# ilias-laoukili/gnn-sparsification-research

Hardware: AMD Instinct MI355X
Metric: scored edges/sec (Jaccard+ApproxER) (higher is better)
Workload: dtype f64; 1 GPU; configs[1] Roman-empire Jaccard+ApproxER; n=22662, E=65854, jl_k=2674, cg_maxiter=500, blas_threads_order=8, rng=device, parallelism=1 GPU

## Files before the change

### gnn-sparsification-research_amd/csrc/gs_cg.hpp

```cpp
#pragma once
#include <algorithm>
#include <climits>
#include <cstddef>
#include <cstdlib>

#include "gs_internal.hpp"

namespace gs {

static constexpr int kMaxChunks = 64;
static constexpr int64_t kStoreQRowLen = 8;

struct ChunkArg {
    int32_t count;
    int64_t a[kMaxChunks];
    int64_t len[kMaxChunks];
};
static_assert(offsetof(ChunkArg, len) == offsetof(ChunkArg, a) + sizeof(int64_t) * kMaxChunks,
              "chunks_to_device copies a and len as one block");

inline ChunkArg make_chunks(int64_t n, int32_t threads) {
    ChunkArg ch{};
    if (n <= 10000 || threads <= 1) {
        ch.count = 1;
// ... 160 lines not shown
    int64_t slots;
    bool slots_forced;
    bool res_unit;
    bool res_dcount;
    bool res_prof;
    bool res_ell;
    bool res_stab;
    bool res_qlds;
    int res_rbw;
    int reg_nt;
    int64_t reg_keep;
    int reg_split;
    bool reg_split_auto;
    int32_t reg_split_spin;
    int reg_window;
};

bool cg_regres_applies(int64_t n, int T, const int64_t *len, int reg_nt);
bool cg_regres_wide(int64_t n, int T, const int64_t *len, int reg_nt);

static constexpr int kRegLayoutChunks = 16;
static constexpr size_t kRegLdsBytes = 160 * 1024;

inline int reg_geometry(int NT, int T, const int64_t *len, int &G) {
    if (T < 1 || 32 * T > NT) return -1;
    G = 1;
    while (G < 8 && 32 * T * (2 * G) <= NT) G *= 2;
    int64_t smax = 0;
    for (int t = 0; t < T; ++t) smax = std::max<int64_t>(smax, (len[t] & ~(int64_t)31) >> 5);
    return (int)((smax + G - 1) / G);
// ... 68 lines not shown
    int64_t zs = 0;
    for (int t = 0; t < T; ++t) {
        L.lbase[t] = zs;
        zs += L.keep[t];
    }
    L.W = W;
    for (int t = 0; t < T && W > 0; ++t) {
        L.wbase[t] = zs;
        zs += W * align;
    }
    L.zslot = zs;
    L.dyn = sizeof(double) * ((size_t)zs + 2 + L.dsl + 6 * (size_t)nch + 2 * kRegLayoutChunks);
    return true;
}

inline CgPlan cg_plan(int64_t n, int64_t lnnz, int64_t ncols, int32_t blas_threads) {
    CgPlan p{};
    if (blas_threads > kMaxChunks) blas_threads = kMaxChunks;
    p.ch = make_chunks(n, blas_threads);
    const ChunkArg &ch = p.ch;

    const char *e;
    p.res_unit = !(e = getenv("GSPARSE_RES_UNIT")) || atoi(e) != 0;
    p.res_dcount = !(e = getenv("GSPARSE_RES_DCOUNT")) || atoi(e) != 0;
    p.res_prof = getenv("GSPARSE_RES_PROF") != nullptr;
    p.res_ell = (e = getenv("GSPARSE_RES_ELL")) && atoi(e) != 0;
    p.res_stab = !(e = getenv("GSPARSE_RES_STAB")) || atoi(e) != 0;
    p.res_qlds = !(e = getenv("GSPARSE_RES_QLDS")) || atoi(e) != 0;
    p.res_rbw = 0;
    if ((e = getenv("GSPARSE_RES_RBW")))
        p.res_rbw = atoi(e) == 44 ? 44 : atoi(e) == 27 ? 27 : atoi(e) == 26 ? 26 : 28;
    p.reg_nt = ((e = getenv("GSPARSE_REG_NT")) && atoi(e) == 256) ? 256 : 512;
    p.reg_keep = (e = getenv("GSPARSE_REG_KEEP")) ? atoll(e) : INT64_MAX;
    p.reg_split = (e = getenv("GSPARSE_REG_SPLIT")) ? atoi(e) : -1;
    p.reg_split_auto = getenv("GSPARSE_REG_SPLIT_AUTO") != nullptr;
    p.reg_split_spin = (e = getenv("GSPARSE_REG_SPLIT_SPIN")) ? atoi(e) : INT32_MIN;
    p.reg_window = -1;
    if ((e = getenv("GSPARSE_REG_WINDOW"))) p.reg_window = atoi(e) == 3 ? 3 : atoi(e) == 4 ? 4 : 0;

    const int64_t waves2 = ((ncols + 127) / 128) * 32 * (int64_t)ch.count;
    p.cpl = waves2 >= 4096 ? 2 : 1;
    if ((e = getenv("GSPARSE_CG_CPL"))) p.cpl = atoi(e) == 1 ? 1 : 2;
    const int64_t ncb = (int32_t)((ncols + 64 * p.cpl - 1) / (64 * p.cpl));

    const bool resident = n > 10000 && n <= 24576 && ch.count >= 4 && lnnz <= kStoreQRowLen * n;
    const bool regres = cg_regres_applies(n, ch.count, ch.len, p.reg_nt);
    const bool regwide = cg_regres_wide(n, ch.count, ch.len, p.reg_nt);
    p.mode = resident && regwide                   ? 5
             : resident                            ? 4
             : (n > 0 && lnnz > kStoreQRowLen * n) ? 3
             : ncols >= 2048                       ? 0
             : ncols >= 512                        ? 1
                                                   : 3;
// ... 49 lines not shown
```

### gnn-sparsification-research_amd/csrc/gs_cg_reg.hip

```cpp
#include "gs_cg.hpp"
#include "gs_cg_reg.hpp"

#ifndef GS_CG_XG
#define GS_CG_XG 0
#endif

namespace gs {

__global__ void k_ell8_count(int32_t n, const int64_t *__restrict__ lp, int64_t *__restrict__ cnt,
                             uint16_t *__restrict__ rlen) {
    for (int64_t i = blockIdx.x * (int64_t)blockDim.x + threadIdx.x; i < n;
         i += (int64_t)gridDim.x * blockDim.x) {
        const int64_t len = lp[i + 1] - lp[i];
        cnt[i] = len > 8 ? len - 8 : 0;
        rlen[i] = (uint16_t)len;
    }
}

__device__ __forceinline__ uint32_t p_code(int32_t c, int32_t i, int T, const int64_t *__restrict__ tab,
                                           int W, int &nwin) {
    if (c < tab[0] || c >= tab[T - 1] + tab[kRegMaxChunks + T - 1]) return 0x8000u | (uint32_t)c;
    int t = 0;
    while (t + 1 < T && c >= tab[t + 1]) ++t;
    const int64_t o = c - tab[t], keep = tab[2 * kRegMaxChunks + t];
    if (o < keep) return (uint32_t)(tab[3 * kRegMaxChunks + t] + o);
    if (W > 0) {
        const int64_t oi = (int64_t)i - tab[t], n32 = tab[kRegMaxChunks + t] & ~(int64_t)31;
        if (oi >= 0 && oi < n32 && o < n32) {
            const int64_t sc = o >> 6, si = oi >> 6;
            if (sc - si <= 1 && si - sc <= 1) {
                ++nwin;
                return (uint32_t)(tab[4 * kRegMaxChunks + t] + ((sc - (keep >> 6)) % W) * 64 + (o & 63));
            }
        }
    }
    return 0x8000u | (uint32_t)c;
}

__device__ __forceinline__ int row_dslot(int32_t c, int T, const int64_t *__restrict__ tab, int G,
                                         int dmul, int32_t d0 = 0) {
    int t = 0;
    while (t + 1 < T && c >= tab[t + 1]) ++t;
// ... 5 lines not shown
    const int tid = (chain / CW) * 64 + (chain % CW) + CW * g;
    if (dmul == 3) {
        const int lb = (int)tab[3 * kRegMaxChunks + t];
        const int s0 = d0 + (tid & ~31);
        return (tid & ~31) + ((lb + (tid & 31) + 1 - s0) & 31);
    }
    return dmul == 2 ? 2 * tid + par : tid;
}

__global__ void k_ell8_fill(int32_t r0, int32_t n, int T, const int64_t *__restrict__ tab, uint32_t pad,
                            int G, int dmul, int32_t dslot0, const int64_t *__restrict__ lp,
                            const int32_t *__restrict__ li, const double *__restrict__ lv,
                            const int64_t *__restrict__ optr, uint4 *__restrict__ ell,
                            double *__restrict__ ellv, uint16_t *__restrict__ ocol,
                            double *__restrict__ oval, uint8_t *__restrict__ rflag, int W,
                            unsigned long long *__restrict__ wcount) {
    for (int64_t i = r0 + blockIdx.x * (int64_t)blockDim.x + threadIdx.x; i < n;
         i += (int64_t)gridDim.x * blockDim.x) {
        const int64_t e0 = lp[i], len = lp[i + 1] - e0;
        const uint32_t dcode = dslot0 >= 0 ? (uint32_t)(dslot0 + row_dslot((int32_t)i, T, tab, G, dmul, dslot0)) : 0u;
        int nwin = 0;
        auto code = [&](int64_t e) -> uint32_t {
            return (dslot0 >= 0 && li[e] == i) ? dcode : p_code(li[e], (int32_t)i, T, tab, W, nwin);
        };
        uint32_t w[4] = {0, 0, 0, 0};
        bool glob = false;
        for (int k = 0; k < 8; ++k) {
            const uint32_t cc = k < len ? code(e0 + k) : pad;
            glob = glob || (cc & 0x8000u) != 0;
            w[k >> 1] |= cc << (16 * (k & 1));
            if (ellv) ellv[i * 8 + k] = k < len ? lv[e0 + k] : 0.0;
        }
        ell[i] = make_uint4(w[0], w[1], w[2], w[3]);
        if (rflag) rflag[i] = (uint8_t)((glob ? 1 : 0) | (len > 8 ? 2 : 0));
        for (int64_t k = 8; k < len; ++k) {
            ocol[optr[i] + k - 8] = (uint16_t)code(e0 + k);
            if (oval) oval[optr[i] + k - 8] = lv[e0 + k];
        }
// ... 32 lines not shown
    hipStream_t s = c->stream;
    const int T = plan.ch.count;
    const int64_t *ha = plan.ch.a, *hlen = plan.ch.len;
    const int64_t slots = plan.slots;
    const bool ufast = unit && dcount;
    RegLayout lay0, layw;
    GS_CHECK(reg_layout(n, plan.ch, plan.reg_nt, plan.reg_keep, ufast, lay0), GS_EUNSUPPORTED,
             "register-resident CG: n=%lld, %d chunks out of range", (long long)n, T);
    const int NT = lay0.NT, G = lay0.G, rsel = lay0.R;
    const int wask = !kRegWindowBuilt ? 0 : plan.reg_window < 0 ? kRegWindowDefault : plan.reg_window;
    const bool have_w = wask > 0 && reg_layout(n, plan.ch, plan.reg_nt, plan.reg_keep, ufast, layw, wask) &&
                        layw.W > 0;
    const bool dbank = GS_CG_V2 && NT == 512 && G == 2 && ufast;
    const int dsl = lay0.dsl;
    const size_t lds_max = kRegLdsBytes;
    double regv = c->er.reg;
    int64_t regbits;
    memcpy(&regbits, &regv, sizeof(regbits));
    std::vector<int64_t> key = {c->g.epoch, regbits, n, T, G, NT, ufast ? 1 : 0, unit, dcount, dbank ? 1 : 0,
                                have_w ? layw.W : 0, plan.reg_window};
    for (int t = 0; t < T; ++t) key.insert(key.end(), {ha[t], hlen[t], lay0.keep[t]});
    auto *ocnt = (int64_t *)c->buf("er_reg_ocnt").ensure(sizeof(int64_t) * (n + 1));
    auto *optr = (int64_t *)c->buf("er_reg_optr").ensure(sizeof(int64_t) * (n + 1));
    auto *rlen = (uint16_t *)c->buf("er_reg_rlen").ensure(sizeof(uint16_t) * n);
    const bool fresh = key != c->reg_ell_key;
    if (fresh) {
        c->reg_ell_key.clear();
        c->reg_split_key.clear();
        GS_HIP(hipMemsetAsync(ocnt, 0, sizeof(int64_t) * (n + 1), s));
        k_ell8_count<<<grid_for(n, 256, 8192), 256, 0, s>>>((int32_t)n, lp, ocnt, rlen);
        exclusive_scan_i64(c, ocnt, optr, n + 1);
        GS_HIP(hipMemcpyAsync(&c->reg_nov, optr + n, sizeof(int64_t), hipMemcpyDeviceToHost, s));
        GS_HIP(hipStreamSynchronize(s));
    }
    const int64_t nov = c->reg_nov;
// ... 3 lines not shown
        host.assign(5 * kRegMaxChunks, 0);
        for (int t = 0; t < T; ++t) {
            host[t] = ha[t];
            host[kRegMaxChunks + t] = hlen[t];
            host[2 * kRegMaxChunks + t] = L.keep[t];
            host[3 * kRegMaxChunks + t] = L.lbase[t];
            host[4 * kRegMaxChunks + t] = L.wbase[t];
        }
        GS_HIP(hipMemcpyAsync(dev, host.data(), kTabBytes, hipMemcpyHostToDevice, s));
    };
    auto *ell = (uint4 *)c->buf("er_reg_ell").ensure(sizeof(uint4) * n);
    auto *rflag = (uint8_t *)c->buf("er_reg_rflag").ensure((size_t)n + 64);
    double *ellv = ufast ? nullptr : (double *)c->buf("er_reg_ellv").ensure(sizeof(double) * 8 * n);
    auto *ocol = (uint16_t *)c->buf("er_reg_ocol").ensure(sizeof(uint16_t) * (nov + 1));
    double *oval = ufast ? nullptr : (double *)c->buf("er_reg_oval").ensure(sizeof(double) * (nov + 1));
    auto fill = [&](const RegLayout &L, const int64_t *dev, unsigned long long *wcount) {
        k_ell8_fill<<<grid_for(n, 256, 8192), 256, 0, s>>>(0, (int32_t)n, T, dev, (uint32_t)L.zslot, G,
                                                          NT == 256 ? 2 : dbank ? 3 : 1,
                                                          ufast ? (int32_t)L.zslot + 2 : -1,
                                                          lp, li, lv, optr, ell, ellv, ocol, oval, rflag, L.W,
                                                          wcount);
        GS_HIP(hipGetLastError());
    };
    if (fresh && have_w) {
        auto *dch2 = (int64_t *)c->buf("er_reg_chunks2").ensure(kTabBytes);
        auto *dcnt = (unsigned long long *)c->buf("er_reg_wcnt").ensure(sizeof(unsigned long long) * 3);
        unsigned long long hcnt[3] = {0, 0, 0};
        GS_HIP(hipMemsetAsync(dcnt, 0, sizeof(hcnt), s));
        upload(lay0, c->reg_hch2, dch2);
        fill(lay0, dch2, nullptr);
        k_reg_slow_slots<<<T, 64, 0, s>>>(T, dch2, rflag, dcnt);
        upload(layw, c->reg_hch, dch);
        fill(layw, dch, dcnt + 2);
        k_reg_slow_slots<<<T, 64, 0, s>>>(T, dch, rflag, dcnt + 1);
        GS_HIP(hipGetLastError());
        GS_HIP(hipMemcpyAsync(hcnt, dcnt, sizeof(hcnt), hipMemcpyDeviceToHost, s));
        GS_HIP(hipStreamSynchronize(s));
        const bool use_w = plan.reg_window > 0 || hcnt[1] < hcnt[0];
        c->reg_win[0] = use_w ? layw.W : 0;
        c->reg_win[1] = (int64_t)hcnt[0];
        c->reg_win[2] = (int64_t)hcnt[1];
        c->reg_win[3] = use_w ? (int64_t)hcnt[2] : 0;
        if (!use_w) {
            upload(lay0, c->reg_hch, dch);
            fill(lay0, dch, nullptr);
        }
        c->reg_ell_key = key;
    } else if (fresh) {
        c->reg_win[0] = 0, c->reg_win[1] = c->reg_win[2] = -1, c->reg_win[3] = 0;
        upload(lay0, c->reg_hch, dch);
        fill(lay0, dch, nullptr);
        c->reg_ell_key = key;
    }
    const RegLayout &lay = (have_w && c->reg_win[0] > 0) ? layw : lay0;
    if (!fresh) upload(lay, c->reg_hch, dch);
    const uint32_t pad = (uint32_t)lay.zslot;
    const size_t dyn = lay.dyn;
    RegArgs A{};
    A.qreg = 0;
    int ncu = 256;
    GS_HIP(hipDeviceGetAttribute(&ncu, hipDeviceAttributeMultiprocessorCount, c->device));
    int P = 0;
    int64_t W = ncols;
    split_abort_poll(c, false);
    if (c->reg_split_off && c->reg_split_off_epoch != c->g.epoch) c->reg_split_off = false;
    if (NT == 512 && T >= 2 && ncols > 0 && !c->reg_split_off) {
// ... 58 lines not shown
    A.oval = oval;
    A.diag = diag;
    A.rflag = rflag;

    A.zslot = (int32_t)pad;
    A.maxiter = maxiter;
    A.rtol = rtol;
    A.iters = iters;
    A.T = T;
    A.ca = dch;
    A.cl = dch + kRegMaxChunks;
    A.ck = dch + 2 * kRegMaxChunks;
    A.cb = dch + 3 * kRegMaxChunks;
    A.cw = dch + 4 * kRegMaxChunks;
    A.W = lay.W;
    A.prof = prof;
    auto launch_whole = [&]() {
        if (W <= 0) return;
        if (NT == 512) {
            if (G == 1) regwide_launch_g1(A, rsel, ufast, dyn, (unsigned)wslots, s);
            else if (G == 2) regwide_launch_g2(A, rsel, ufast, dyn, (unsigned)wslots, s);
            else if (G == 4) regwide_launch_g4(A, rsel, ufast, dyn, (unsigned)wslots, s);
            else regwide_launch_g8(A, rsel, ufast, dyn, (unsigned)wslots, s);
        } else if (G == 1) regres_launch_g1(A, rsel, ufast, dyn, (unsigned)wslots, s);
        else if (G == 2) regres_launch_g2(A, rsel, ufast, dyn, (unsigned)wslots, s);
        else if (G == 4) regres_launch_g4(A, rsel, ufast, dyn, (unsigned)wslots, s);
        else regres_launch_g8(A, rsel, ufast, dyn, (unsigned)wslots, s);
        GS_HIP(hipGetLastError());
    };
    if (P < 2) {
// ... 31 lines not shown
    GS_HIP(hipMemcpyAsync(dpt, c->reg_split_hpt.data(), sizeof(hpt), hipMemcpyHostToDevice, s));
    GS_HIP(hipMemcpyAsync(dtab, c->reg_split_htab.data(), sizeof(htab), hipMemcpyHostToDevice, s));
    auto *ells = (uint4 *)c->buf("er_reg_split_ell").ensure(sizeof(uint4) * n);
    double *ellvs = ufast ? nullptr : (double *)c->buf("er_reg_split_ellv").ensure(sizeof(double) * 8 * n);
    auto *ocols = (uint16_t *)c->buf("er_reg_split_ocol").ensure(sizeof(uint16_t) * (nov + 1));
    double *ovals = ufast ? nullptr : (double *)c->buf("er_reg_split_oval").ensure(sizeof(double) * (nov + 1));
    std::vector<int64_t> skey = {P, Gs};
    skey.insert(skey.end(), pc0, pc0 + P + 1);
    const bool sfresh = skey != c->reg_split_key;
    for (int h = 0; h < P && sfresh; ++h) {
        const int32_t r0 = (int32_t)ha[pc0[h]];
        const int32_t r1 = (int32_t)(ha[pc0[h + 1] - 1] + hlen[pc0[h + 1] - 1]);
        const int32_t zsh = hpt[h * kRegPartTab + 4 * kRegMaxChunks + 1];
        k_ell8_fill<<<grid_for(r1 - r0, 256, 8192), 256, 0, s>>>(
            r0, r1, pc0[h + 1] - pc0[h], dtab + h * 4 * kRegMaxChunks, (uint32_t)zsh, Gs, 1,
            ufast ? zsh + 2 : -1, lp, li, lv, optr, ells, ellvs, ocols, ovals, nullptr, 0, nullptr);
        GS_HIP(hipGetLastError());
    }
    c->reg_split_key = skey;
    double *pgs = (double *)c->buf("er_reg_split_pg").ensure(sizeof(double) * (size_t)groups * 2 * ldn);
    double *xch = (double *)c->buf("er_reg_split_xch").ensure(sizeof(double) * (size_t)groups * 2 * kRegMaxChunks);
    auto *flg = (int32_t *)c->buf("er_reg_split_flags").ensure(sizeof(int32_t) * ((size_t)groups * P + 1));
    GS_HIP(hipMemsetAsync(flg, 0, sizeof(int32_t) * ((size_t)groups * P + 1), s));
    RegArgs B = A;
    B.col0 = col0 + W;
    B.ncols = tailn;
    B.Xc = Xc + W * ldn;
    B.pg = pgs;
    B.ell = ells;
    B.ellv = ellvs;
    B.ocol = ocols;
    B.oval = ovals;
    B.prof = nullptr;
    B.P = P;
    B.ptab = dpt;
    B.xch = xch;
    B.flags = flg;
    B.abortf = flg + (size_t)groups * P;
    int wclk_khz = 100000;
    GS_HIP(hipDeviceGetAttribute(&wclk_khz, hipDeviceAttributeWallClockRate, c->device));
    B.spinmax = 20 * std::max(wclk_khz, 1);
    if (plan.reg_split_spin != INT32_MIN) B.spinmax = plan.reg_split_spin;
    const unsigned grid = (unsigned)(groups * P);
    launch_whole();
    if (Gs == 4) regwide_split_launch_g4(B, Rs, ufast, dyns, grid, s);
    else regwide_split_launch_g8(B, Rs, ufast, dyns, grid, s);
    GS_HIP(hipGetLastError());
    RegArgs Cw = A;
    Cw.col0 = col0 + W;
// ... 54 lines not shown
```

### gnn-sparsification-research_amd/csrc/gs_cg_reg.hpp

```cpp
#pragma once
#include <algorithm>

#include "gs_internal.hpp"

namespace gs {

static constexpr int kRegThreads = 512;
static constexpr int kRegMaxChunks = kRegThreads / 32;
#ifndef GS_KPRE
#define GS_KPRE 1
#endif
static constexpr int kPre = GS_KPRE;
#ifndef GS_KPRE_P
#define GS_KPRE_P GS_KPRE
#endif
static constexpr int kPreP = GS_KPRE_P;
#ifndef GS_CG_V2
#define GS_CG_V2 1
#endif
#ifndef GS_PGRP
#define GS_PGRP 4
#endif
#ifndef GS_P1S
#define GS_P1S 1
// ... 27 lines not shown
    const int64_t *ca, *cl;
    const int64_t *ck, *cb;
    long long *prof;
    int32_t qreg;
    int32_t P;
    const int32_t *ptab;
    double *xch;
    int32_t *flags;
    int32_t *abortf;
    int32_t spinmax;
    const double *diag;
    const uint8_t *rflag;
    const int32_t *gate;
    int32_t W;
    const int64_t *cw;
};
#ifndef GS_CG_QS
#define GS_CG_QS 1
#endif
#ifndef GS_CG_XG
#define GS_CG_XG 0
#endif
static constexpr bool kRegWindowBuilt = GS_CG_V2 && GS_CG_QS && !GS_CG_XG;
static constexpr int kRegWindowDefault = 3;
static constexpr int kRegPartTab = 4 * kRegMaxChunks + 4;

struct AgD {
    uint32_t lo, hi;
};
__device__ __forceinline__ double ag_get(const AgD &a) {
// ... 470 lines not shown
```

### gnn-sparsification-research_amd/csrc/gs_cg_wide.hpp

```cpp
#pragma once
#include "gs_cg_reg.hpp"

#ifndef GS_CG_QS
#define GS_CG_QS 1
#endif
#ifndef GS_CG_QPRE
#define GS_CG_QPRE 8
#endif
#ifndef GS_CG_QAUX
#define GS_CG_QAUX 2
#endif
#ifndef GS_CG_XAUX
#define GS_CG_XAUX 0
#endif
#ifndef GS_CG_XG
#define GS_CG_XG 0
#endif

namespace gs {

template <int HI>
__device__ __forceinline__ uint32_t wide_code_addr(uint32_t w) {
    uint32_t a;
    if (HI)
// ... 16 lines not shown
__device__ __forceinline__ double wide_readlane(double v, int ln) {
    const uint64_t b = (uint64_t)__double_as_longlong(v);
    const uint32_t lo = (uint32_t)__builtin_amdgcn_readlane((int)(uint32_t)b, ln);
    const uint32_t hi = (uint32_t)__builtin_amdgcn_readlane((int)(uint32_t)(b >> 32), ln);
    return __longlong_as_double((long long)(((uint64_t)hi << 32) | lo));
}

template <int G, int R, bool UNIT, bool QR, bool SPLIT = false, bool WIN = false>
__global__ void __launch_bounds__(kRegThreads) k_cg_regwide(RegArgs A) {
    constexpr int CW = 64 / G;
    constexpr bool V2 = GS_CG_V2 && UNIT && !SPLIT;
    constexpr bool DBANK = V2 && G == 2;
    constexpr bool QS = GS_CG_QS && !QR && !SPLIT;
    constexpr bool QSX = GS_CG_XG && QR && !SPLIT;
    constexpr bool P1 = GS_P1S && WIN;
    static_assert(!WIN || (V2 && G == 2 && QS),
                  "the p window: whole columns, unit form, two threads per chain, q stored");
    extern __shared__ double lds[];
    const int part = SPLIT ? (int)(blockIdx.x % (unsigned)A.P) : 0;
    const int group = SPLIT ? (int)(blockIdx.x / (unsigned)A.P) : (int)blockIdx.x;
    const int ngroups = SPLIT ? (int)(gridDim.x / (unsigned)A.P) : (int)gridDim.x;
    const int32_t *ptab = SPLIT ? A.ptab + part * kRegPartTab : nullptr;
    const int T = SPLIT ? ptab[4 * kRegMaxChunks] : A.T, nch = 32 * T;
    const int zslot = SPLIT ? ptab[4 * kRegMaxChunks + 1] : A.zslot;
    const int t0g = SPLIT ? ptab[4 * kRegMaxChunks + 2] : 0;
    const int Tg = SPLIT ? A.T : T;
    double *sp = lds;
    double *acc_pq = lds + zslot + 2 + (UNIT ? kRegThreads : 0), *acc_rr = acc_pq + nch;
    double *side_p = acc_pq + 2 * nch, *side_q = acc_pq + 3 * nch, *side_r = acc_pq + 4 * nch;
    double *side_x = acc_pq + 5 * nch;
// ... 14 lines not shown
    const int chain = (tid >> 6) * CW + jj;
    const bool live = chain < nch;
    const int t = live ? chain >> 5 : 0, j = chain & 31;
    const int L = s_ch[kRegMaxChunks + t];
    const int n32 = L & ~31;
    const int S = live ? n32 >> 5 : -1;
    const int tl = L - n32;
    int base = s_ch[t] + j + 32 * g;
    int uc = S > g ? (S - g + G - 1) / G : 0;
    const bool tail = live && g == 0 && j < tl;
    const int trow = s_ch[t] + n32 + j;
    const int tix = t * 32 + j;
    int ulds = 0;
    uint64_t gmask = 0, lmask = 0;
    uint32_t wdelta = 0, wbytes = 0;
    auto launder = [&]() {
        asm volatile("" : "+v"(base), "+v"(uc), "+s"(ulds));
        if constexpr (V2) asm volatile("" : "+s"(gmask), "+s"(lmask));
        if constexpr (WIN) asm volatile("" : "+s"(wdelta), "+s"(wbytes));
    };
    auto chunk_num = [&](int v) { return WIN ? __builtin_amdgcn_readfirstlane(v) : v; };
    const int ca_t = chunk_num(s_ch[t]), keep_t = chunk_num(s_ch[2 * kRegMaxChunks + t]),
              lbase_t = chunk_num(s_ch[3 * kRegMaxChunks + t]);
    {
        int uk = R;
        if (live) {
            const int o0 = base - ca_t;
            uk = keep_t > o0 ? (keep_t - o0 + 32 * G - 1) / (32 * G) : 0;
        }
        for (int off = 32; off >= 1; off >>= 1) uk = min(uk, __shfl_xor(uk, off, 64));
        ulds = __builtin_amdgcn_readfirstlane(uk);
    }
    auto lds0 = [&]() -> uint32_t { return (uint32_t)(lbase_t + base - ca_t) * 8u; };
    if constexpr (WIN) {
// ... 10 lines not shown
    constexpr int kOob = (int)0x80000000;
    constexpr int kAux = SPLIT ? 16 : 0;
    int poff = 0;
    auto vm_drain = [] { __builtin_amdgcn_s_waitcnt(0x0f70); };
    const __amdgpu_buffer_rsrc_t ers =
        __builtin_amdgcn_make_buffer_rsrc((void *)A.ell, 0, (int)(A.n * 16), 0x00020000);
    const __amdgpu_buffer_rsrc_t lrs =
        __builtin_amdgcn_make_buffer_rsrc((void *)A.rlen, 0, (int)(A.n * 2), 0x00020000);
    const __amdgpu_buffer_rsrc_t drs =
        __builtin_amdgcn_make_buffer_rsrc((void *)(V2 ? A.diag : nullptr), 0, (int)(V2 ? A.n * 8 : 0),
                                          0x00020000);
    if (tid == 0) spl[zslot] = 0.0;

    auto code_of = [&](int row) {
        const int o = row - ca_t;
        return o < keep_t ? lbase_t + o : 0x8000 | row;
    };
    auto ldc = [&](int cd) -> double {
        double v = spl[cd < 0x8000 ? cd : zslot];
        if (__builtin_amdgcn_ballot_w64(cd >= 0x8000)) {
            const double vg = __builtin_bit_cast(
                double, __builtin_amdgcn_raw_buffer_load_b64(prs, cd < 0x8000 ? kOob : (cd & 0x7fff) * 8 + poff, 0, kAux));
            v = cd < 0x8000 ? v : vg;
            vm_drain();
        }
        return v;
    };
    auto stc = [&](int cd, double v) {
        spl[cd < 0x8000 ? cd : zslot + 1] = v;
        if (__builtin_amdgcn_ballot_w64(cd >= 0x8000))
            __builtin_amdgcn_raw_buffer_store_b64(
// ... 361 lines not shown
                __builtin_bit_cast(__attribute__((ext_vector_type(2))) unsigned, v), xrs,
                valid(u) ? base * 8 : kOob, 256 * G * u, GS_CG_QAUX);
        };
        {
            launder();
            double acc = 0.0;
#pragma unroll
            for (int u = 0; u < R; ++u) {
                if constexpr (!QR) x[u] = 0.0;
                else qr[u] = 0.0;
                r[u] = valid(u) ? A.Rr[(int64_t)rowof(u) * A.ld + c] : 0.0;
                chain_step(acc, r[u], r[u], u, true);
            }
            if (g == 0 && live) acc_rr[chain] = acc;
            if (tail) {
                side_r[tix] = A.Rr[(int64_t)trow * A.ld + c];
                side_x[tix] = 0.0;
            }
        }
        __syncthreads();
        double rr = finish(acc_rr, side_r, side_r);
        const double bn = __builtin_sqrt(rr);
        const double atol = A.rtol * bn;
        int32_t done = 0;
        double rho_prev = 0.0, alpha_prev = 0.0;
        const bool act = !(bn == 0.0) && !(__builtin_sqrt(rr) < atol);
        for (int32_t it = 0; act && it < A.maxiter; ++it) {
            if (it > 0 && __builtin_sqrt(rr) < atol) break;
            const double rho_cur = rr;
            const double beta = it > 0 ? rho_cur / rho_prev : 0.0;
            if constexpr (SPLIT) poff = (it & 1) * (int)A.ldn * 8;
// ... 230 lines not shown
                            wq = wq == wbytes ? 0u : wq;
                        }
                    } else if constexpr (V2) {
                        if (valid(u)) qv = spmv2(rowof(u), eb[u], db[u], pv, u, pnx, png);
                    } else if (valid(u)) qv = spmv(rowof(u), eb[u], lb[u], pv, u);
                    if constexpr (QSX) q2store(u, qv);
                    else if constexpr (QR) qr[u] = qv;
                    if constexpr (QS) qstore(u, qv);
                    chain_step(acc, pv, qv, u);
                    __builtin_amdgcn_sched_barrier(0);
                }
                if (g == 0 && live) acc_pq[chain] = acc;
                if (tail) {
                    double pt;
                    side_q[tix] = spmv(trow, A.ell[trow], (int)A.rlen[trow], pt, -1);
                    side_p[tix] = pt;
                }
            }
            __syncthreads();
            lap(1);
            const double pq = finish(acc_pq, side_p, side_q);
            const double alpha = rho_cur / pq;
            lap(2);
            if constexpr (QSX) {
                launder();
                double acc = 0.0;
                constexpr int kPq = GS_CG_QPRE;
                double qb[R], xb[R], pgb[R];
                auto pre = [&](int u) {
                    qb[u] = q2load(u);
                    xb[u] = it > 0 ? xload2(u) : 0.0;
// ... 236 lines not shown
```

### gnn-sparsification-research_amd/csrc/gs_er.hip

```cpp
#include "gs_cg.hpp"
#include "gs_pairwise.hpp"

namespace gs {

__global__ void k_upper_flags(const int32_t *__restrict__ rows, const int32_t *__restrict__ ix,
                              int64_t nnz, int64_t *__restrict__ flag) {
    for (int64_t e = blockIdx.x * (int64_t)blockDim.x + threadIdx.x; e < nnz;
         e += (int64_t)gridDim.x * blockDim.x)
        flag[e] = rows[e] < ix[e] ? 1 : 0;
}

__global__ void k_edge_ids(const int64_t *__restrict__ flag, const int64_t *__restrict__ pos,
                           int64_t nnz, int64_t *__restrict__ eid) {
    for (int64_t e = blockIdx.x * (int64_t)blockDim.x + threadIdx.x; e < nnz;
         e += (int64_t)gridDim.x * blockDim.x)
        eid[e] = flag[e] ? pos[e] : -1;
}

__global__ void k_b_counts(const int64_t *__restrict__ ip, const int32_t *__restrict__ ix,
                           const int64_t *__restrict__ tp, const int32_t *__restrict__ ti,
                           int64_t n, int64_t *__restrict__ cnt) {
    for (int64_t i = blockIdx.x * (int64_t)blockDim.x + threadIdx.x; i < n;
         i += (int64_t)gridDim.x * blockDim.x) {
        int64_t c = 0;
// ... 393 lines not shown
            out[8 + 32 + t] = L.keep[t];
            out[8 + 48 + t] = L.lbase[t];
            out[8 + 64 + t] = L.wbase[t];
        }
    });
}

int gs_er_reg_window(gs_ctx *c, int64_t out[4]) {
    return guard([&] {
        GS_CHECK(c, GS_EINVAL, "null context");
        GS_CHECK(out, GS_EINVAL, "out is NULL");
        std::copy(c->reg_win, c->reg_win + 4, out);
    });
}

int gs_er_scores(gs_ctx *c, int64_t col0, int64_t col1, int64_t e0, int64_t e1, int finalize,
                 double *out, int loc) {
    return guard([&] {
        GS_CHECK(c, GS_EINVAL, "null context");
        ErState &er = c->er;
        GS_CHECK(er.solved, GS_ESTATE, "gs_er_solve first");
        GS_CHECK(0 <= col0 && col0 <= col1 && col1 <= er.k, GS_EINVAL, "bad column range");
        GS_CHECK(0 <= e0 && e0 <= e1 && e1 <= c->g.nnz, GS_EINVAL, "bad edge range");
        GS_CHECK(er_cols_solved(er, col0, col1), GS_ESTATE,
                 "columns [%lld, %lld) were not all solved since gs_er_prepare", (long long)col0,
                 (long long)col1);
        GS_HIP(hipSetDevice(c->device));
        int64_t cnt = e1 - e0;
        double *dout = (double *)out_device(c, c->outbuf, out, sizeof(double) * cnt, loc);
        if (cnt) {
// ... 68 lines not shown
```

### gnn-sparsification-research_amd/csrc/gs_internal.hpp

```cpp
#pragma once

#include <hip/hip_runtime.h>

#include <algorithm>
#include <cstdint>
#include <cstdio>
#include <cstring>
#include <map>
#include <memory>
#include <string>
#include <vector>

#include "../../include/gsparse.h"

namespace gs {

void set_error(const char *fmt, ...);

struct GsError {
    int code;
};

#define GS_HIP(expr)                                                                        \
    do {                                                                                    \
// ... 114 lines not shown
    std::map<std::string, gs::ProfEntry> prof;
    std::vector<std::string> prof_order;
    std::vector<gs::ProfPending> pending;
    gs::Graph g;
    gs::ErState er;
    std::vector<uint64_t> zig_key;
    int64_t zig_draws = 0;
    gs::DevBuf scratch[6];
    gs::DevBuf outbuf, inbuf, inbuf2;
    std::map<std::string, gs::DevBuf> named;
    std::vector<int64_t> reg_ell_key, reg_split_key;
    int64_t reg_nov = 0;
    std::vector<int64_t> reg_hch;
    std::vector<int64_t> reg_hch2;
    int64_t reg_win[4] = {0, -1, -1, 0};
    bool reg_split_off = false;
    int64_t reg_split_off_epoch = -1;
    std::vector<int32_t> reg_split_hpt;
    std::vector<int64_t> reg_split_htab;
    int32_t *split_abort_host = nullptr;
    hipEvent_t split_abort_ev = nullptr;
    bool split_abort_pending = false;
    int split_abort_parts = 0;
    int64_t split_aborts = 0;
    std::shared_ptr<gs::BbRun> bb;
    std::shared_ptr<gs::JacState> jac;
    void *truss_host = nullptr;
    gs::DevBuf &buf(const char *name) { return named[name]; }
};

// ... 45 lines not shown
```

### gnn-sparsification-research_amd/gsparse/_lib.py

```python

from __future__ import annotations

import ctypes
import os
import threading

import numpy as np

_HERE = os.path.dirname(os.path.abspath(__file__))
LIB_PATH = os.environ.get("GSPARSE_LIB", os.path.join(_HERE, "libgsparse.so"))

GS_HOST, GS_DEVICE = 0, 1
GS_OK, GS_EINVAL, GS_EHIP, GS_ENOMEM, GS_ESTATE, GS_EUNSUPPORTED, GS_EINDEX = 0, -1, -2, -3, -4, -5, -6
GS_ENOCONV = -7

_i64 = ctypes.c_int64
_i32 = ctypes.c_int32
_u64 = ctypes.c_uint64
_f64 = ctypes.c_double
_vp = ctypes.c_void_p
_int = ctypes.c_int

SIGNATURES = {
    "gs_api_version": (_int, []),
# ... 26 lines not shown
    "gs_feature_cosine_f64": (_int, [_vp, _vp, _i64, _int, _i64, _i64, _vp, _int]),
    "gs_er_prepare": (_int, [_vp, _i64, _f64, ctypes.POINTER(_i64)]),
    "gs_er_project_rows": (_int, [_vp, _i64, _i64, _vp, _int, _f64]),
    "gs_er_project_pcg64": (_int, [_vp, _u64, _u64, _u64, _u64, _f64]),
    "gs_er_project_pcg64_cols": (_int, [_vp, _u64, _u64, _u64, _u64, _f64, _i64, _i64]),
    "gs_er_project_rows_cols": (_int, [_vp, _i64, _i64, _vp, _int, _f64, _i64, _i64]),
    "gs_er_solve": (_int, [_vp, _i64, _i64, _i32, _f64, _i32]),
    "gs_er_scores": (_int, [_vp, _i64, _i64, _i64, _i64, _int, _vp, _int]),
    "gs_er_iterations": (_int, [_vp, _vp, _int]),
    "gs_er_copy_z": (_int, [_vp, _i64, _i64, _vp, _int]),
    "gs_er_split": (_int, [_i64, _i32, _vp]),
    "gs_er_plan": (_int, [_i64, _i64, _i64, _i32, _vp]),
    "gs_er_reg_layout": (_int, [_i64, _i32, _i32, _vp]),
    "gs_er_reg_layout_w": (_int, [_i64, _i32, _i32, _i32, _vp]),
    "gs_er_reg_window": (_int, [_vp, _vp]),
    "gs_topk_mask": (_int, [_vp, _vp, _int, _i64, _i64, _i64, _int, _vp, _int,
                            ctypes.POINTER(_f64), ctypes.POINTER(_i64), ctypes.POINTER(_i64)]),
    "gs_segment_argmax": (_int, [_vp, _vp, _int, _i64, _vp, _int, _i64, _i64, _vp, _int]),
    "gs_segment_topk": (_int, [_vp, _vp, _int, _i64, _vp, _int, _i64, _i64, _i64, _vp, _int, _vp,
                               _int, ctypes.POINTER(_i64), ctypes.POINTER(_i64), _vp, _int]),
    "gs_sample_mask": (_int, [_vp, _vp, _int, _i64, _i64, _i64, _u64, _u64, _u64, _u64, _vp, _int,
                              ctypes.POINTER(_i32), ctypes.POINTER(_i64), ctypes.POINTER(_i64)]),
    "gs_pcg64_doubles": (_int, [_vp, _u64, _u64, _u64, _u64, _u64, _i64, _vp, _int]),
    "gs_sample_probs": (_int, [_vp, _vp, _int, _i64, _vp, _int, ctypes.POINTER(_f64)]),
    "gs_cumsum_ordered": (_int, [_vp, _vp, _int, _i64, _vp, _int]),
    "gs_undirected_ids": (_int, [_vp, _i64, _i64, _vp, _vp, _int, _vp, _int, ctypes.POINTER(_i64),
                                 ctypes.POINTER(_i32)]),
    "gs_random_mask": (_int, [_vp, _vp, _int, _i64, _i64, _vp, _int, _i64, _vp, _int,
                              ctypes.POINTER(_f64), ctypes.POINTER(_i64), ctypes.POINTER(_i64),
                              ctypes.POINTER(_i64)]),
# ... 267 lines not shown
```

### gnn-sparsification-research_amd/gsparse/engine.py

```python

from __future__ import annotations

import ctypes
import os
import queue
import threading

import numpy as np

from . import _args as A
from ._lib import GS_DEVICE, GS_HOST, Context, ptr
from .plans import (OPENBLAS_MAX_THREADS, aa_weights, bb_geometry,
                    blas_threads_default, er_plan, er_reg_layout, er_reg_layout_w, er_split,
                    jl_dim, xer_sparse_plan)

_ROW_CHUNK_BYTES = 64 << 20


class Engine:

    def __init__(self, ctx: Context):
        self.ctx = ctx
        self.n, self.nnz, self.symmetric = ctx.shape()
        self._indptr = None

    def indptr(self) -> np.ndarray:
        if self._indptr is None:
            ip = np.empty(self.n + 1, dtype=np.int64)
            self.ctx.call("gs_graph_copy_csr", ptr(ip), None, None, GS_HOST)
# ... 166 lines not shown
                  e1: int | None = None, out=None):
        e1 = self.nnz if e1 is None else e1
        o, loc = self._scores_out(e1 - e0, out)
        self.ctx.call("gs_er_scores", col0, col1, e0, e1, int(finalize), ptr(o), loc)
        return o

    def er_iterations(self) -> np.ndarray:
        it = np.empty(self.k, dtype=np.int32)
        self.ctx.call("gs_er_iterations", ptr(it), GS_HOST)
        return it

    def er_reg_window(self) -> dict:
        o = np.zeros(4, dtype=np.int64)
        self.ctx.call("gs_er_reg_window", ptr(o))
        return dict(zip(("W", "slow_plain", "slow_window", "window_codes"), o.tolist()))

    def er_z(self, col0: int, col1: int) -> np.ndarray:
        z = np.empty((self.n, col1 - col0), dtype=np.float64)
        self.ctx.call("gs_er_copy_z", col0, col1, ptr(z), GS_HOST)
        return z

    def approx_er(self, epsilon: float = 0.3, seed: int = 42, max_cg_iters: int = 500,
                  cg_tol: float = 1e-6, blas_threads: int | None = None,
                  rng_mode: str | None = None):
        rng = np.random.default_rng(seed)
        n = self.n
        k = jl_dim(n, epsilon)
        m = self.er_prepare(k)
        if m == 0:
            return np.zeros(self.nnz, dtype=np.float64)
# ... 279 lines not shown
```

### gnn-sparsification-research_amd/gsparse/plans.py

```python

from __future__ import annotations

import os

import numpy as np

from . import _lib
from ._lib import ptr


def blas_threads_default() -> int:
    return min(_blas_threads_requested(), OPENBLAS_MAX_THREADS)


OPENBLAS_MAX_THREADS = 64


def _blas_threads_requested() -> int:
    env = os.environ.get("GSPARSE_BLAS_THREADS")
    if env:
        return max(1, int(env))
    try:
        from threadpoolctl import threadpool_info

# ... 43 lines not shown


def er_reg_layout_w(n: int, blas_threads: int, window: int, unit: bool = True) -> dict | None:
    o = np.zeros(88, dtype=np.int64)
    _lib.check(_lib.lib().gs_er_reg_layout_w(n, blas_threads, int(bool(unit)), int(window), ptr(o)),
               "gs_er_reg_layout_w")
    if o[0] == 0:
        return None
    d = dict(zip(("threads", "G", "R", "T", "zslot", "dsl", "lds_bytes", "W"), o[:8].tolist()))
    T = d["T"]
    for i, name in enumerate(("start", "len", "keep", "lbase", "wbase")):
        d[name] = o[8 + 16 * i:8 + 16 * i + T].tolist()
    return d


def xer_sparse_plan(n: int, cus: int = 0) -> dict:
    o = np.zeros(4, dtype=np.int64)
    _lib.check(_lib.lib().gs_xer_sparse_plan(int(n), int(cus), ptr(o)), "gs_xer_sparse_plan")
    return dict(zip(("batch", "budget_bytes", "chunks", "chunk_rows"), o.tolist()))


def bb_geometry(n: int, nsrc: int, nranks: int = 1, lpart: int = 0) -> dict:
    o = np.zeros(7, dtype=np.int64)
    _lib.check(_lib.lib().gs_bb_geometry(n, nsrc, nranks, lpart, ptr(o)), "gs_bb_geometry")
    return dict(zip(("K", "lm_coop", "lm_W", "S", "threads", "nbatch", "slabs"), o.tolist()))
```

### include/gsparse.h

```cpp
#ifndef GSPARSE_H
#define GSPARSE_H

#include <stdint.h>

#ifdef __cplusplus
extern "C" {
#endif

#define GS_API_VERSION 3

enum {
    GS_OK = 0,
    GS_EINVAL = -1,
    GS_EHIP = -2,
    GS_ENOMEM = -3,
    GS_ESTATE = -4,
    GS_EUNSUPPORTED = -5,
    GS_EINDEX = -6,
    GS_ENOCONV = -7
};

enum { GS_HOST = 0, GS_DEVICE = 1 };

typedef struct gs_ctx gs_ctx;
// ... 59 lines not shown
                            double sqrt_k, int64_t col0, int64_t col1);
int gs_er_solve(gs_ctx *ctx, int64_t col0, int64_t col1, int32_t maxiter, double rtol,
                int32_t blas_threads);
int gs_er_scores(gs_ctx *ctx, int64_t col0, int64_t col1, int64_t e0, int64_t e1,
                 int finalize, double *out, int loc);
int gs_er_iterations(gs_ctx *ctx, int32_t *iters, int loc);
int gs_er_copy_z(gs_ctx *ctx, int64_t col0, int64_t col1, double *out, int loc);
int gs_er_split(int64_t k, int32_t parts, int64_t *bounds);
int gs_er_plan(int64_t n, int64_t lnnz, int64_t ncols, int32_t blas_threads, int32_t out[4]);
int gs_er_reg_layout(int64_t n, int32_t blas_threads, int32_t unit, int64_t out[72]);

int gs_er_reg_layout_w(int64_t n, int32_t blas_threads, int32_t unit, int32_t window, int64_t out[88]);

int gs_er_reg_window(gs_ctx *c, int64_t out[4]);

int gs_topk_mask(gs_ctx *ctx, const double *scores, int s_loc, int64_t nnz, int64_t E,
                 int64_t num_keep, int keep_lowest, uint8_t *mask, int m_loc,
                 double *cut, int64_t *n_beyond, int64_t *n_tied);

int gs_segment_argmax(gs_ctx *ctx, const double *scores, int s_loc, int64_t nscores,
                      const int64_t *src, int src_loc, int64_t E, int64_t n, int64_t *pick,
                      int pick_loc);

enum { GS_SEGK_EMPTY = 0, GS_SEGK_ALL, GS_SEGK_SHORT, GS_SEGK_LDS, GS_SEGK_STREAM, GS_SEGK_CLASSES };
int gs_segment_topk(gs_ctx *ctx, const double *scores, int s_loc, int64_t nscores,
                    const int64_t *src, int src_loc, int64_t E, int64_t n, int64_t k,
                    uint8_t *mask, int mask_loc, uint8_t *status, int status_loc,
                    int64_t *n_guaranteed, int64_t *n_ambiguous, int64_t *class_counts,
                    int ncounts);

// ... 118 lines not shown
```

Before: 472,300 scored edges/s.

## Home chunk tail rows in LDS slots for register-resident CG SpMV

Gives the per-chunk tail rows (beyond the 32-aligned part) of the register-resident CG a fixed home in the LDS side buffers. The ELL column codes for those rows now point at LDS instead of falling back to global memory. This is meant to cut slow global gathers of p during SpMV. The cost is extra encoding paths in code_of and p_code, an extra fill and slow-slot count at setup, and a check that the tail slots fit within the LDS code range.

```diff
diff --git a/gnn-sparsification-research_amd/csrc/gs_cg.hpp b/gnn-sparsification-research_amd/csrc/gs_cg.hpp
--- a/gnn-sparsification-research_amd/csrc/gs_cg.hpp
+++ b/gnn-sparsification-research_amd/csrc/gs_cg.hpp
@@ -198,6 +198,7 @@
     bool reg_split_auto;
     int32_t reg_split_spin;
     int reg_window;
+    bool reg_tailhome;
 };
 
 bool cg_regres_applies(int64_t n, int T, const int64_t *len, int reg_nt);
@@ -296,6 +297,10 @@
     return true;
 }
 
+inline int64_t reg_tail_base(const RegLayout &L) {
+    return L.NT == 512 ? L.zslot + 2 + L.dsl + 2 * 32 * (int64_t)L.T : -1;
+}
+
 inline CgPlan cg_plan(int64_t n, int64_t lnnz, int64_t ncols, int32_t blas_threads) {
     CgPlan p{};
     if (blas_threads > kMaxChunks) blas_threads = kMaxChunks;
@@ -319,6 +324,7 @@
     p.reg_split_spin = (e = getenv("GSPARSE_REG_SPLIT_SPIN")) ? atoi(e) : INT32_MIN;
     p.reg_window = -1;
     if ((e = getenv("GSPARSE_REG_WINDOW"))) p.reg_window = atoi(e) == 3 ? 3 : atoi(e) == 4 ? 4 : 0;
+    p.reg_tailhome = !(e = getenv("GSPARSE_REG_TAILHOME")) || atoi(e) != 0;
 
     const int64_t waves2 = ((ncols + 127) / 128) * 32 * (int64_t)ch.count;
     p.cpl = waves2 >= 4096 ? 2 : 1;
diff --git a/gnn-sparsification-research_amd/csrc/gs_cg_reg.hip b/gnn-sparsification-research_amd/csrc/gs_cg_reg.hip
--- a/gnn-sparsification-research_amd/csrc/gs_cg_reg.hip
+++ b/gnn-sparsification-research_amd/csrc/gs_cg_reg.hip
@@ -18,14 +18,16 @@
 }
 
 __device__ __forceinline__ uint32_t p_code(int32_t c, int32_t i, int T, const int64_t *__restrict__ tab,
-                                           int W, int &nwin) {
+                                           int W, int &nwin, int32_t tb) {
     if (c < tab[0] || c >= tab[T - 1] + tab[kRegMaxChunks + T - 1]) return 0x8000u | (uint32_t)c;
     int t = 0;
     while (t + 1 < T && c >= tab[t + 1]) ++t;
     const int64_t o = c - tab[t], keep = tab[2 * kRegMaxChunks + t];
     if (o < keep) return (uint32_t)(tab[3 * kRegMaxChunks + t] + o);
+    const int64_t n32 = tab[kRegMaxChunks + t] & ~(int64_t)31;
+    if (tb >= 0 && o >= n32) return (uint32_t)(tb + 32 * t + (o - n32));
     if (W > 0) {
-        const int64_t oi = (int64_t)i - tab[t], n32 = tab[kRegMaxChunks + t] & ~(int64_t)31;
+        const int64_t oi = (int64_t)i - tab[t];
         if (oi >= 0 && oi < n32 && o < n32) {
             const int64_t sc = o >> 6, si = oi >> 6;
             if (sc - si <= 1 && si - sc <= 1) {
@@ -61,14 +63,14 @@
                             const int64_t *__restrict__ optr, uint4 *__restrict__ ell,
                             double *__restrict__ ellv, uint16_t *__restrict__ ocol,
                             double *__restrict__ oval, uint8_t *__restrict__ rflag, int W,
-                            unsigned long long *__restrict__ wcount) {
+                            unsigned long long *__restrict__ wcount, int32_t tbase) {
     for (int64_t i = r0 + blockIdx.x * (int64_t)blockDim.x + threadIdx.x; i < n;
          i += (int64_t)gridDim.x * blockDim.x) {
         const int64_t e0 = lp[i], len = lp[i + 1] - e0;
         const uint32_t dcode = dslot0 >= 0 ? (uint32_t)(dslot0 + row_dslot((int32_t)i, T, tab, G, dmul, dslot0)) : 0u;
         int nwin = 0;
         auto code = [&](int64_t e) -> uint32_t {
-            return (dslot0 >= 0 && li[e] == i) ? dcode : p_code(li[e], (int32_t)i, T, tab, W, nwin);
+            return (dslot0 >= 0 && li[e] == i) ? dcode : p_code(li[e], (int32_t)i, T, tab, W, nwin, tbase);
         };
         uint32_t w[4] = {0, 0, 0, 0};
         bool glob = false;
@@ -131,11 +133,18 @@
     const bool dbank = GS_CG_V2 && NT == 512 && G == 2 && ufast;
     const int dsl = lay0.dsl;
     const size_t lds_max = kRegLdsBytes;
+    const bool th = plan.reg_tailhome && NT == 512;
+    auto tail_base = [&](const RegLayout &L) -> int32_t {
+        const int64_t b = th ? reg_tail_base(L) : -1;
+        GS_CHECK(b + 32 * (int64_t)T <= 0x8000 && (size_t)(b + 32 * (int64_t)T) * 8 <= L.dyn, GS_EUNSUPPORTED,
+                 "register-resident CG: tail slots %lld.. outside the LDS codes", (long long)b);
+        return (int32_t)b;
+    };
     double regv = c->er.reg;
     int64_t regbits;
     memcpy(&regbits, &regv, sizeof(regbits));
     std::vector<int64_t> key = {c->g.epoch, regbits, n, T, G, NT, ufast ? 1 : 0, unit, dcount, dbank ? 1 : 0,
-                                have_w ? layw.W : 0, plan.reg_window};
+                                have_w ? layw.W : 0, plan.reg_window, th ? 1 : 0};
     for (int t = 0; t < T; ++t) key.insert(key.end(), {ha[t], hlen[t], lay0.keep[t]});
     auto *ocnt = (int64_t *)c->buf("er_reg_ocnt").ensure(sizeof(int64_t) * (n + 1));
     auto *optr = (int64_t *)c->buf("er_reg_optr").ensure(sizeof(int64_t) * (n + 1));
@@ -169,24 +178,35 @@
     double *ellv = ufast ? nullptr : (double *)c->buf("er_reg_ellv").ensure(sizeof(double) * 8 * n);
     auto *ocol = (uint16_t *)c->buf("er_reg_ocol").ensure(sizeof(uint16_t) * (nov + 1));
     double *oval = ufast ? nullptr : (double *)c->buf("er_reg_oval").ensure(sizeof(double) * (nov + 1));
-    auto fill = [&](const RegLayout &L, const int64_t *dev, unsigned long long *wcount) {
+    auto fill = [&](const RegLayout &L, const int64_t *dev, unsigned long long *wcount, int32_t tb) {
         k_ell8_fill<<<grid_for(n, 256, 8192), 256, 0, s>>>(0, (int32_t)n, T, dev, (uint32_t)L.zslot, G,
                                                           NT == 256 ? 2 : dbank ? 3 : 1,
                                                           ufast ? (int32_t)L.zslot + 2 : -1,
                                                           lp, li, lv, optr, ell, ellv, ocol, oval, rflag, L.W,
-                                                          wcount);
+                                                          wcount, tb);
         GS_HIP(hipGetLastError());
+    };
+    auto *dcnt = (unsigned long long *)c->buf("er_reg_wcnt").ensure(sizeof(unsigned long long) * 4);
+    auto final_fill = [&](const RegLayout &L) {
+        unsigned long long slow = 0;
+        fill(L, dch, nullptr, tail_base(L));
+        GS_HIP(hipMemsetAsync(dcnt + 3, 0, sizeof(slow), s));
+        k_reg_slow_slots<<<T, 64, 0, s>>>(T, dch, rflag, dcnt + 3);
+        GS_HIP(hipGetLastError());
+        GS_HIP(hipMemcpyAsync(&slow, dcnt + 3, sizeof(slow), hipMemcpyDeviceToHost, s));
+        GS_HIP(hipStreamSynchronize(s));
+        c->reg_th[0] = th ? 1 : 0;
+        c->reg_th[1] = (int64_t)slow;
     };
     if (fresh && have_w) {
         auto *dch2 = (int64_t *)c->buf("er_reg_chunks2").ensure(kTabBytes);
-        auto *dcnt = (unsigned long long *)c->buf("er_reg_wcnt").ensure(sizeof(unsigned long long) * 3);
         unsigned long long hcnt[3] = {0, 0, 0};
         GS_HIP(hipMemsetAsync(dcnt, 0, sizeof(hcnt), s));
         upload(lay0, c->reg_hch2, dch2);
-        fill(lay0, dch2, nullptr);
+        fill(lay0, dch2, nullptr, -1);
         k_reg_slow_slots<<<T, 64, 0, s>>>(T, dch2, rflag, dcnt);
         upload(layw, c->reg_hch, dch);
-        fill(layw, dch, dcnt + 2);
+        fill(layw, dch, dcnt + 2, -1);
         k_reg_slow_slots<<<T, 64, 0, s>>>(T, dch, rflag, dcnt + 1);
         GS_HIP(hipGetLastError());
         GS_HIP(hipMemcpyAsync(hcnt, dcnt, sizeof(hcnt), hipMemcpyDeviceToHost, s));
@@ -196,15 +216,18 @@
         c->reg_win[1] = (int64_t)hcnt[0];
         c->reg_win[2] = (int64_t)hcnt[1];
         c->reg_win[3] = use_w ? (int64_t)hcnt[2] : 0;
-        if (!use_w) {
-            upload(lay0, c->reg_hch, dch);
-            fill(lay0, dch, nullptr);
+        if (!use_w) upload(lay0, c->reg_hch, dch);
+        if (th || !use_w) {
+            final_fill(use_w ? layw : lay0);
+        } else {
+            c->reg_th[0] = 0;
+            c->reg_th[1] = (int64_t)hcnt[1];
         }
         c->reg_ell_key = key;
     } else if (fresh) {
         c->reg_win[0] = 0, c->reg_win[1] = c->reg_win[2] = -1, c->reg_win[3] = 0;
         upload(lay0, c->reg_hch, dch);
-        fill(lay0, dch, nullptr);
+        final_fill(lay0);
         c->reg_ell_key = key;
     }
     const RegLayout &lay = (have_w && c->reg_win[0] > 0) ? layw : lay0;
@@ -293,6 +316,7 @@
     A.cb = dch + 3 * kRegMaxChunks;
     A.cw = dch + 4 * kRegMaxChunks;
     A.W = lay.W;
+    A.tbase = c->reg_th[0] ? tail_base(lay) : -1;
     A.prof = prof;
     auto launch_whole = [&]() {
         if (W <= 0) return;
@@ -354,7 +378,7 @@
         const int32_t zsh = hpt[h * kRegPartTab + 4 * kRegMaxChunks + 1];
         k_ell8_fill<<<grid_for(r1 - r0, 256, 8192), 256, 0, s>>>(
             r0, r1, pc0[h + 1] - pc0[h], dtab + h * 4 * kRegMaxChunks, (uint32_t)zsh, Gs, 1,
-            ufast ? zsh + 2 : -1, lp, li, lv, optr, ells, ellvs, ocols, ovals, nullptr, 0, nullptr);
+            ufast ? zsh + 2 : -1, lp, li, lv, optr, ells, ellvs, ocols, ovals, nullptr, 0, nullptr, -1);
         GS_HIP(hipGetLastError());
     }
     c->reg_split_key = skey;
@@ -373,6 +397,7 @@
     B.oval = ovals;
     B.prof = nullptr;
     B.P = P;
+    B.tbase = -1;
     B.ptab = dpt;
     B.xch = xch;
     B.flags = flg;
diff --git a/gnn-sparsification-research_amd/csrc/gs_cg_reg.hpp b/gnn-sparsification-research_amd/csrc/gs_cg_reg.hpp
--- a/gnn-sparsification-research_amd/csrc/gs_cg_reg.hpp
+++ b/gnn-sparsification-research_amd/csrc/gs_cg_reg.hpp
@@ -65,6 +65,7 @@
     const int32_t *gate;
     int32_t W;
     const int64_t *cw;
+    int32_t tbase;
 };
 #ifndef GS_CG_QS
 #define GS_CG_QS 1
diff --git a/gnn-sparsification-research_amd/csrc/gs_cg_wide.hpp b/gnn-sparsification-research_amd/csrc/gs_cg_wide.hpp
--- a/gnn-sparsification-research_amd/csrc/gs_cg_wide.hpp
+++ b/gnn-sparsification-research_amd/csrc/gs_cg_wide.hpp
@@ -54,6 +54,7 @@
     constexpr bool QS = GS_CG_QS && !QR && !SPLIT;
     constexpr bool QSX = GS_CG_XG && QR && !SPLIT;
     constexpr bool P1 = GS_P1S && WIN;
+    constexpr bool TH = !SPLIT;
     static_assert(!WIN || (V2 && G == 2 && QS),
                   "the p window: whole columns, unit form, two threads per chain, q stored");
     extern __shared__ double lds[];
@@ -98,10 +99,18 @@
     int ulds = 0;
     uint64_t gmask = 0, lmask = 0;
     uint32_t wdelta = 0, wbytes = 0;
+    int tn32 = 0x7fffffff, tdelta = 0;
+    const bool thome = TH && A.tbase >= 0;
+    if constexpr (WIN) {
+        if (thome) {
+            tn32 = __builtin_amdgcn_readfirstlane(n32);
+            tdelta = __builtin_amdgcn_readfirstlane(A.tbase + 32 * t - n32);
+        }
+    }
     auto launder = [&]() {
         asm volatile("" : "+v"(base), "+v"(uc), "+s"(ulds));
         if constexpr (V2) asm volatile("" : "+s"(gmask), "+s"(lmask));
-        if constexpr (WIN) asm volatile("" : "+s"(wdelta), "+s"(wbytes));
+        if constexpr (WIN) asm volatile("" : "+s"(wdelta), "+s"(wbytes), "+s"(tn32), "+s"(tdelta));
     };
     auto chunk_num = [&](int v) { return WIN ? __builtin_amdgcn_readfirstlane(v) : v; };
     const int ca_t = chunk_num(s_ch[t]), keep_t = chunk_num(s_ch[2 * kRegMaxChunks + t]),
@@ -142,7 +151,11 @@
 
     auto code_of = [&](int row) {
         const int o = row - ca_t;
-        return o < keep_t ? lbase_t + o : 0x8000 | row;
+        if constexpr (WIN) return o < keep_t ? lbase_t + o : o >= tn32 ? tdelta + o : 0x8000 | row;
+        else if constexpr (TH)
+            return o < keep_t ? lbase_t + o
+                   : thome && row >= trow - (tix & 31) ? A.tbase + tix + (row - trow) : 0x8000 | row;
+        else return o < keep_t ? lbase_t + o : 0x8000 | row;
     };
     auto ldc = [&](int cd) -> double {
         double v = spl[cd < 0x8000 ? cd : zslot];
@@ -534,7 +547,9 @@
             }
             if (g == 0 && live) acc_rr[chain] = acc;
             if (tail) {
-                side_r[tix] = A.Rr[(int64_t)trow * A.ld + c];
+                int tr = trow;
+                asm volatile("" : "+v"(tr));
+                side_r[tix] = A.Rr[(int64_t)tr * A.ld + c];
                 side_x[tix] = 0.0;
             }
         }
@@ -795,7 +810,7 @@
                 if (tail) {
                     double pt;
                     side_q[tix] = spmv(trow, A.ell[trow], (int)A.rlen[trow], pt, -1);
-                    side_p[tix] = pt;
+                    if (!thome || trow - ca_t < keep_t) side_p[tix] = pt;
                 }
             }
             __syncthreads();
diff --git a/gnn-sparsification-research_amd/csrc/gs_er.hip b/gnn-sparsification-research_amd/csrc/gs_er.hip
--- a/gnn-sparsification-research_amd/csrc/gs_er.hip
+++ b/gnn-sparsification-research_amd/csrc/gs_er.hip
@@ -431,6 +431,26 @@
     });
 }
 
+int gs_er_reg_tail_base(int64_t n, int32_t blas_threads, int32_t unit, int32_t window, int64_t *out) {
+    return guard([&] {
+        GS_CHECK(out, GS_EINVAL, "out is NULL");
+        GS_CHECK(n >= 0, GS_EINVAL, "negative size");
+        *out = -1;
+        const CgPlan plan = cg_plan(n, 0, 1, blas_threads);
+        RegLayout L;
+        if (!reg_layout(n, plan.ch, plan.reg_nt, plan.reg_keep, unit != 0, L, window)) return;
+        *out = reg_tail_base(L);
+    });
+}
+
+int gs_er_reg_tail_home(gs_ctx *c, int64_t out[2]) {
+    return guard([&] {
+        GS_CHECK(c, GS_EINVAL, "null context");
+        GS_CHECK(out, GS_EINVAL, "out is NULL");
+        std::copy(c->reg_th, c->reg_th + 2, out);
+    });
+}
+
 int gs_er_scores(gs_ctx *c, int64_t col0, int64_t col1, int64_t e0, int64_t e1, int finalize,
                  double *out, int loc) {
     return guard([&] {
diff --git a/gnn-sparsification-research_amd/csrc/gs_internal.hpp b/gnn-sparsification-research_amd/csrc/gs_internal.hpp
--- a/gnn-sparsification-research_amd/csrc/gs_internal.hpp
+++ b/gnn-sparsification-research_amd/csrc/gs_internal.hpp
@@ -152,6 +152,7 @@
     std::vector<int64_t> reg_hch;
     std::vector<int64_t> reg_hch2;
     int64_t reg_win[4] = {0, -1, -1, 0};
+    int64_t reg_th[2] = {0, -1};
     bool reg_split_off = false;
     int64_t reg_split_off_epoch = -1;
     std::vector<int32_t> reg_split_hpt;
diff --git a/gnn-sparsification-research_amd/gsparse/_lib.py b/gnn-sparsification-research_amd/gsparse/_lib.py
--- a/gnn-sparsification-research_amd/gsparse/_lib.py
+++ b/gnn-sparsification-research_amd/gsparse/_lib.py
@@ -64,6 +64,8 @@
     "gs_er_reg_layout": (_int, [_i64, _i32, _i32, _vp]),
     "gs_er_reg_layout_w": (_int, [_i64, _i32, _i32, _i32, _vp]),
     "gs_er_reg_window": (_int, [_vp, _vp]),
+    "gs_er_reg_tail_base": (_int, [_i64, _i32, _i32, _i32, _vp]),
+    "gs_er_reg_tail_home": (_int, [_vp, _vp]),
     "gs_topk_mask": (_int, [_vp, _vp, _int, _i64, _i64, _i64, _int, _vp, _int,
                             ctypes.POINTER(_f64), ctypes.POINTER(_i64), ctypes.POINTER(_i64)]),
     "gs_segment_argmax": (_int, [_vp, _vp, _int, _i64, _vp, _int, _i64, _i64, _vp, _int]),
diff --git a/gnn-sparsification-research_amd/gsparse/engine.py b/gnn-sparsification-research_amd/gsparse/engine.py
--- a/gnn-sparsification-research_amd/gsparse/engine.py
+++ b/gnn-sparsification-research_amd/gsparse/engine.py
@@ -11,8 +11,8 @@
 from . import _args as A
 from ._lib import GS_DEVICE, GS_HOST, Context, ptr
 from .plans import (OPENBLAS_MAX_THREADS, aa_weights, bb_geometry,
-                    blas_threads_default, er_plan, er_reg_layout, er_reg_layout_w, er_split,
-                    jl_dim, xer_sparse_plan)
+                    blas_threads_default, er_plan, er_reg_layout, er_reg_layout_w, er_reg_tail_base,
+                    er_split, jl_dim, xer_sparse_plan)
 
 _ROW_CHUNK_BYTES = 64 << 20
 
@@ -209,6 +209,11 @@
         o = np.zeros(4, dtype=np.int64)
         self.ctx.call("gs_er_reg_window", ptr(o))
         return dict(zip(("W", "slow_plain", "slow_window", "window_codes"), o.tolist()))
+
+    def er_reg_tail_home(self) -> dict:
+        o = np.zeros(2, dtype=np.int64)
+        self.ctx.call("gs_er_reg_tail_home", ptr(o))
+        return {"on": bool(o[0]), "slow": int(o[1])}
 
     def er_z(self, col0: int, col1: int) -> np.ndarray:
         z = np.empty((self.n, col1 - col0), dtype=np.float64)
diff --git a/gnn-sparsification-research_amd/gsparse/plans.py b/gnn-sparsification-research_amd/gsparse/plans.py
--- a/gnn-sparsification-research_amd/gsparse/plans.py
+++ b/gnn-sparsification-research_amd/gsparse/plans.py
@@ -81,6 +81,13 @@
     return d
 
 
+def er_reg_tail_base(n: int, blas_threads: int, unit: bool = True, window: int = 0) -> int:
+    o = np.zeros(1, dtype=np.int64)
+    _lib.check(_lib.lib().gs_er_reg_tail_base(n, blas_threads, int(bool(unit)), int(window), ptr(o)),
+               "gs_er_reg_tail_base")
+    return int(o[0])
+
+
 def xer_sparse_plan(n: int, cus: int = 0) -> dict:
     o = np.zeros(4, dtype=np.int64)
     _lib.check(_lib.lib().gs_xer_sparse_plan(int(n), int(cus), ptr(o)), "gs_xer_sparse_plan")
diff --git a/include/gsparse.h b/include/gsparse.h
--- a/include/gsparse.h
+++ b/include/gsparse.h
@@ -97,6 +97,10 @@
 
 int gs_er_reg_window(gs_ctx *c, int64_t out[4]);
 
+int gs_er_reg_tail_base(int64_t n, int32_t blas_threads, int32_t unit, int32_t window, int64_t *out);
+
+int gs_er_reg_tail_home(gs_ctx *c, int64_t out[2]);
+
 int gs_topk_mask(gs_ctx *ctx, const double *scores, int s_loc, int64_t nnz, int64_t E,
                  int64_t num_keep, int keep_lowest, uint8_t *mask, int m_loc,
                  double *cut, int64_t *n_beyond, int64_t *n_tied);
```

Result: no change. 474,900 scored edges/s, median of 5 (+0.5%).
